# Joao-M-Silva/padel_analytics

Hardware: NVIDIA H100
Metric: frames/sec through trackers.runner (all 4 trackers) (higher is better)
Workload: dtype f16 storage, f32 accumulate

## Files before the change

padel_analytics_b200/csrc/api.cu:

```cuda
#include <atomic>
#include <cstring>
#include <map>
#include <memory>
#include <mutex>
#include <vector>

#include "internal.h"

namespace pb {

static thread_local std::string g_error;
std::atomic<long long> g_launches{0};

void set_error(const char* fmt, ...) {
  char buf[1024];
  va_list ap;
  va_start(ap, fmt);
  vsnprintf(buf, sizeof(buf), fmt, ap);
  va_end(ap);
  g_error = buf;
}

static std::atomic<int> g_plan_sm_limit{0};
static std::atomic<int> g_plan_pdl{-1};
// ... 145 lines not shown
  return -1;
}

int pb_program_op_info(const pb_program* p, int i, pb_op_info* out) {
  PB_CHECK(p && out, "program_op_info: null argument");
  PB_CHECK(i >= 0 && i < (int)p->ops.size(), "program_op_info: op %d out of range", i);
  const Op& op = p->ops[i];
  memset(out, 0, sizeof(*out));
  out->kernel = pb_program_op_kernel(p, i);
  if (op.kind == OpKind::Conv) {
    const ConvPlan& pl = *op.conv;
    const ConvKParams& kp = pl.kp;
    const pb_conv_desc& d = pl.desc;
    out->desc = d;
    out->variant = pl.variant != 1                ? PB_CONV_PER_TAP
                   : d.in_layout == PB_IN_STEM4   ? PB_CONV_STEM
                   : d.ksize == 1                 ? PB_CONV_HALO_1X1
                   : d.stride == 2                ? PB_CONV_HALO_S2
                                                  : PB_CONV_HALO;
    out->epi = pl.epi;
    out->BN = kp.BN;
    out->n_ntiles = kp.n_ntiles;
    out->KB = kp.KB;
    out->kblocks = kp.kblocks;
    if (pl.variant == 1) {
      out->S = kp.hs_S;
      out->G = kp.hs_G;
      out->b_resident = kp.b_resident;
      out->a_stages = kp.a_stages;
      out->b_stages = kp.b_stages;
      out->tma_store = kp.st_bytes != 0;
      out->st_pool = kp.st_pool;
    } else {
      out->S = 1;
      out->G = 1;
      out->a_stages = out->b_stages = kp.stages;
    }
    out->grid = pl.grid;
    out->total_tiles = kp.total_tiles;
    out->pdl = pl.pdl;
  } else {
    out->in = op.in;
    out->out = op.out;
    out->N = op.N;
    out->H = op.H;
    out->W = op.W;
    out->C = op.C;
    out->c_off = op.c_off;
    out->c = op.c;
    out->out_C = op.out_C;
    out->out_coff = op.out_coff;
    out->weight = op.hw;
    out->bias = op.hb;
  }
  return 0;
}

int pb_program_run_range(pb_program* p, int first, int last, void* stream) {
  PB_CHECK(p != nullptr, "program_run: null");
  PB_CHECK(first >= 0 && last <= (int)p->ops.size() && first <= last, "program_run: bad range");
  cudaStream_t s = static_cast<cudaStream_t>(stream);
  for (int i = first; i < last; ++i) {
    const Op& op = p->ops[i];
    int rc = 0;
    switch (op.kind) {
      case OpKind::Conv: rc = conv_plan_launch(op.conv.get(), s); break;
      case OpKind::MaxPool2:
        rc = launch_maxpool2(op.in, op.N, op.H, op.W, op.C, op.c_off, op.c, op.out, op.out_C, op.out_coff, s);
// ... 20 lines not shown
```

padel_analytics_b200/csrc/conv_tc.cu:

```cuda
#include <cstdlib>
#include <cstring>
#include <mutex>

#include "internal.h"
#include "ptx.cuh"
#include "conv_common.cuh"

namespace pb {

constexpr size_t kConvStageBudget = 196 * 1024;

struct ConvSmemTail {
  uint64_t full[kConvMaxStages];
  uint64_t empty[kConvMaxStages];
  float bias[kConvMaxCout];
  float scratch[kConvConsumerWarps * kEpiScratchFloats];
};

struct TileCoord {
  int nt, tw, th, tn;
};
__device__ __forceinline__ TileCoord decode_tile(const ConvKParams& kp, int tile) {
  TileCoord c;
  int t;
  fast_divmod(t, c.nt, tile, kp.fd_nt);
  fast_divmod(t, c.tw, t, kp.fd_w);
  fast_divmod(c.tn, c.th, t, kp.fd_h);
  return c;
}

template <int kEpi>
__global__ void __launch_bounds__(kConvThreads, 1)
conv_tc_kernel(const __grid_constant__ CUtensorMap tmap_a, const __grid_constant__ CUtensorMap tmap_w,
               const __grid_constant__ ConvKParams kp) {
  extern __shared__ __align__(1024) uint8_t smem_raw[];
  uint8_t* smem = smem_raw + ((1024u - (smem_u32(smem_raw) & 1023u)) & 1023u);
  const uint32_t stage_bytes = kp.a_bytes + kp.b_bytes;
  ConvSmemTail* tail = reinterpret_cast<ConvSmemTail*>(smem + (size_t)kp.stages * stage_bytes);

  const int warp = threadIdx.x >> 5;
  const int lane = threadIdx.x & 31;
  const int k_iters = kp.taps * kp.kblocks;

  if (warp == 0 && lane == 0) {
    tma_prefetch_desc(&tmap_a);
    for (int i = 0; i < kp.stages; ++i) {
      mbar_init(&tail->full[i], 2);
      mbar_init(&tail->empty[i], kConvConsumerWarps);
    }
    fence_mbar_init();
  }
  if (warp == 1 && lane == 0) tma_prefetch_desc(&tmap_w);
  for (int i = threadIdx.x; i < kp.cout_pad; i += blockDim.x) tail->bias[i] = kp.bias[i];
  __syncthreads();
  griddep_launch_dependents();
  if (warp != 1) griddep_wait();

  if (warp < 4) {
    warpgroup_reg_dealloc<kConvProducerRegs>();
    if (warp == 0 && lane == 0) {
      int stage = 0;
      uint32_t phase = 0;
      const int TW = 1 << kp.tw_log2, TH = 1 << kp.th_log2;
      const int TN = 128 >> (kp.tw_log2 + kp.th_log2);
      for (int tile = blockIdx.x; tile < kp.total_tiles; tile += gridDim.x) {
        const TileCoord tc = decode_tile(kp, tile);
        for (int tap = 0; tap < kp.taps; ++tap) {
          const int cw = tc.tw * TW + kp.tap_dw[tap];
          const int ch = tc.th * TH + kp.tap_dh[tap];
          const int cc = kp.c_in_off + kp.tap_dc[tap];
          for (int kb = 0; kb < kp.kblocks; ++kb) {
            mbar_wait(&tail->empty[stage], phase ^ 1);
            mbar_arrive_expect_tx(&tail->full[stage], kp.a_bytes);
            tma_load_5d(smem + (size_t)stage * stage_bytes, &tmap_a, &tail->full[stage], cc + kb * kp.KB, cw,
                        kp.tap_d2[tap], ch, tc.tn * TN);
            if (++stage == kp.stages) {
              stage = 0;
              phase ^= 1;
            }
          }
        }
      }
    } else if (warp == 1 && lane == 0) {
      int stage = 0;
      uint32_t phase = 0;
      for (int tile = blockIdx.x; tile < kp.total_tiles; tile += gridDim.x) {
        int nt, tq;
        fast_divmod(tq, nt, tile, kp.fd_nt);
        for (int tap = 0; tap < kp.taps; ++tap) {
          for (int kb = 0; kb < kp.kblocks; ++kb) {
            mbar_wait(&tail->empty[stage], phase ^ 1);
            mbar_arrive_expect_tx(&tail->full[stage], kp.b_tx_bytes);
            tma_load_3d(smem + (size_t)stage * stage_bytes + kp.a_bytes, &tmap_w, &tail->full[stage], kb * kp.KB,
                        nt * kp.BN, tap);
            if (++stage == kp.stages) {
              stage = 0;
              phase ^= 1;
            }
          }
        }
      }
    }
    return;
  }

  warpgroup_reg_alloc<kConvConsumerRegs>();
  const int cw = warp - 4, g = cw >> 2, wq = cw & 3;
  float* scr = tail->scratch + cw * kEpiScratchFloats;
  const uint32_t row_bytes = (uint32_t)kp.KB * 2u;
  const int ksteps = kp.KB / 16;
  const int p = 64 * g + 16 * wq + (lane & 15);
  const int TWm = (1 << kp.tw_log2) - 1, THm = (1 << kp.th_log2) - 1;
  const int tw_i = p & TWm;
  const int th_i = (p >> kp.tw_log2) & THm;
  const int tn_i = p >> (kp.tw_log2 + kp.th_log2);
  float acc[kConvAccRegs];
#pragma unroll
  for (int i = 0; i < kConvAccRegs; ++i) acc[i] = 0.f;
  int stage = 0;
  uint32_t phase = 0;
  for (int tile = blockIdx.x; tile < kp.total_tiles; tile += gridDim.x) {
    const TileCoord tc = decode_tile(kp, tile);
    int prev = -1;
    for (int it = 0; it < k_iters; ++it) {
      mbar_wait(&tail->full[stage], phase);
      const uint32_t a_addr = smem_u32(smem + (size_t)stage * stage_bytes) + 64u * (uint32_t)g * row_bytes;
      const uint64_t adesc = wgmma_desc_kmajor(a_addr, row_bytes);
      const uint64_t bdesc = wgmma_desc_kmajor(smem_u32(smem + (size_t)stage * stage_bytes + kp.a_bytes), row_bytes);
      wgmma_fence();
      for (int k = 0; k < ksteps; ++k)
        mma_group<1, 1>(kp.BN, acc, adesc + (uint64_t)(2 * k), 0, bdesc + (uint64_t)(2 * k), (uint32_t)((it | k) != 0));
      wgmma_commit();
      if (prev >= 0) {
        wgmma_wait<1>();
        consumer_release(&tail->empty[prev], lane);
      }
      prev = stage;
      if (++stage == kp.stages) {
        stage = 0;
        phase ^= 1;
      }
    }
    wgmma_wait<0>();
    wgmma_fence_operands(acc);
    consumer_release(&tail->empty[prev], lane);

    EpiPix px;
    px.ow = (tc.tw << kp.tw_log2) + tw_i;
    px.oh = (tc.th << kp.th_log2) + th_i;
    px.n = tc.tn * (128 >> (kp.tw_log2 + kp.th_log2)) + tn_i;
    px.valid = (px.ow < kp.Wo) && (px.oh < kp.Ho) && (px.n < kp.N);
    px.pix = ((size_t)px.n * kp.Ho + px.oh) * kp.Wo + px.ow;
    epilogue_tile<kEpi>(kp, acc, 1, tc.nt, tail->bias + tc.nt * kp.BN, scr, lane, [&](int, bool& pool_writer) {
      pool_writer = false;
      return px;
    });
  }
}

static EncodeTiledFn get_encode_fn() {
  static EncodeTiledFn fn = nullptr;
  static std::once_flag once;
  std::call_once(once, [] {
    void* p = nullptr;
    cudaDriverEntryPointQueryResult q;
    if (cudaGetDriverEntryPoint("cuTensorMapEncodeTiled", &p, cudaEnableDefault, &q) == cudaSuccess &&
        q == cudaDriverEntryPointSuccess)
      fn = reinterpret_cast<EncodeTiledFn>(p);
  });
  return fn;
}

static int ilog2(int v) {
  int l = 0;
  while ((1 << l) < v) ++l;
  return l;
}

int conv_epi_class(const pb_conv_desc* d, const ConvKParams& kp) {
  static const int enabled = [] {
    const char* e = getenv("PADEL_B200_CONV_EPI");
    return e ? atoi(e) : 1;
  }();
  if (!enabled || kp.dbg_flags != 0) return PB_EPI_GENERIC;
  if (d->head_n != 0 || d->out2_mode != PB_OUT2_NONE || (reinterpret_cast<uintptr_t>(d->out) & 31) != 0)
    return PB_EPI_GENERIC;
  if (d->out_mode == PB_OUT_F32_NHWC) {
// ... 78 lines not shown
  kp.res_first = d->res_before_act ? 1 : 0;
  kp.out = d->out;
  kp.out_C = d->out_C;
  kp.out_coff = d->out_coff;
  kp.out_mode = d->out_mode;
  kp.cout_store = d->cout_store;
  kp.out2 = d->out2;
  kp.out2_C = d->out2_C;
  kp.out2_coff = d->out2_coff;
  kp.out2_mode = d->out2_mode;
  kp.head_w = d->head_weight;
  kp.head_b = d->head_bias;
  kp.head_n = d->head_n;
  kp.head_out = d->head_out;
  {
    const char* df = getenv("PADEL_B200_CONV_DEBUG");
    kp.dbg_flags = df ? atoi(df) : 0;
  }
  plan->variant = 0;
  plan->pdl = plan_pdl();
  plan->epi = conv_epi_class(d, kp);
  if (stem) return conv_stem_setup(d, plan, encode);
  {
    const char* e = getenv("PADEL_B200_CONV_HALO");
    const int mode = e ? atoi(e) : 2;
    const bool s1_3x3 = d->ksize == 3 && d->stride == 1;
    if (mode == 1 || (mode == 2 && (d->cout_pad <= 192 || s1_3x3))) {
      const int rc = d->ksize == 1    ? conv_halo_1x1_setup(d, plan, encode)
                     : d->stride == 2 ? conv_halo_s2_setup(d, plan, encode)
                                      : conv_halo_setup(d, plan, encode, mode == 1 || d->out2_mode == PB_OUT2_POOL2);
      if (rc >= 0) return rc;
    }
  }
  PB_CHECK(d->out2_mode != PB_OUT2_POOL2,
           "conv: PB_OUT2_POOL2 is only implemented by the halo kernel (3x3 stride 1, cout <= 256 or a multiple of 128)");
  int nn = (d->cout_pad + 255) / 256;
  while (d->cout_pad % nn != 0 || (d->cout_pad / nn) % 16 != 0) ++nn;
  kp.n_ntiles = nn;
  kp.BN = d->cout_pad / nn;
  PB_CHECK(kp.BN >= 16 && kp.BN <= 256, "conv: cannot tile cout_pad %d", d->cout_pad);

  long best_cost = -1;
  int best_tw = 0, best_th = 0;
  for (int twl = 7; twl >= 2; --twl) {
    for (int thl = 7 - twl; thl >= 0; --thl) {
      const int TW = 1 << twl, TH = 1 << thl, TN = 128 >> (twl + thl);
      const long cost = (long)((kp.Wo + TW - 1) / TW) * ((kp.Ho + TH - 1) / TH) * ((kp.N + TN - 1) / TN);
      if (best_cost < 0 || cost < best_cost) {
        best_cost = cost;
        best_tw = twl;
        best_th = thl;
      }
    }
  }
  kp.tw_log2 = best_tw;
  kp.th_log2 = best_th;
  const int TW = 1 << best_tw, TH = 1 << best_th, TN = 128 >> (best_tw + best_th);
  kp.tiles_w = (kp.Wo + TW - 1) / TW;
  kp.tiles_h = (kp.Ho + TH - 1) / TH;
  kp.tiles_n = (kp.N + TN - 1) / TN;
  kp.total_tiles = kp.tiles_w * kp.tiles_h * kp.tiles_n * kp.n_ntiles;
  (void)ilog2;

  for (int r = 0; r < d->ksize; ++r)
    for (int q = 0; q < d->ksize; ++q) {
      const int t = r * d->ksize + q;
      const int dy = r - d->ksize / 2, dx = q - d->ksize / 2;
      if (s == 1) {
        kp.tap_dc[t] = 0;
        kp.tap_dw[t] = dx;
        kp.tap_d2[t] = 0;
        kp.tap_dh[t] = dy;
      } else {
        kp.tap_dw[t] = (dx < 0) ? -1 : 0;
        kp.tap_dc[t] = (dx != 0) ? d->C : 0;
        kp.tap_dh[t] = (dy < 0) ? -1 : 0;
        kp.tap_d2[t] = (dy != 0) ? 1 : 0;
      }
    }
  kp.a_bytes = 128u * kp.KB * 2u;
  kp.b_tx_bytes = (uint32_t)kp.BN * kp.KB * 2u;
  kp.b_bytes = (kp.b_tx_bytes + 1023u) & ~1023u;
  const uint32_t stage_bytes = kp.a_bytes + kp.b_bytes;
  int stages = (int)(kConvStageBudget / stage_bytes);
  if (stages > kConvMaxStages) stages = kConvMaxStages;
  PB_CHECK(stages >= 2, "conv: stage too large (%u bytes)", stage_bytes);
  kp.stages = stages;
  plan->smem_bytes = (size_t)stages * stage_bytes + sizeof(ConvSmemTail) + 1024;
  plan->threads = kConvThreads;
  plan->grid = kp.total_tiles < num_sms() ? kp.total_tiles : num_sms();
  const CUtensorMapSwizzle swz = kp.KB == 64   ? CU_TENSOR_MAP_SWIZZLE_128B
                                 : kp.KB == 32 ? CU_TENSOR_MAP_SWIZZLE_64B
                                               : CU_TENSOR_MAP_SWIZZLE_32B;
  {
    const cuuint64_t C = (cuuint64_t)d->C, W = (cuuint64_t)d->W, H = (cuuint64_t)d->H;
    cuuint64_t dims[5];
    cuuint64_t strides[4];
    if (s == 1) {
      dims[0] = C; dims[1] = W; dims[2] = 1; dims[3] = H; dims[4] = (cuuint64_t)d->N;
      strides[0] = C * 2; strides[1] = W * C * 2; strides[2] = W * C * 2; strides[3] = H * W * C * 2;
    } else {
      dims[0] = 2 * C; dims[1] = W / 2; dims[2] = 2; dims[3] = H / 2; dims[4] = (cuuint64_t)d->N;
      strides[0] = 2 * C * 2; strides[1] = W * C * 2; strides[2] = 2 * W * C * 2; strides[3] = H * W * C * 2;
    }
    cuuint32_t box[5] = {(cuuint32_t)kp.KB, (cuuint32_t)TW, 1, (cuuint32_t)TH, (cuuint32_t)TN};
    cuuint32_t estr[5] = {1, 1, 1, 1, 1};
    CUresult r = encode(&plan->tmap_a, CU_TENSOR_MAP_DATA_TYPE_FLOAT16, 5, const_cast<void*>(d->in), dims, strides,
                        box, estr, CU_TENSOR_MAP_INTERLEAVE_NONE, swz, CU_TENSOR_MAP_L2_PROMOTION_L2_128B,
                        CU_TENSOR_MAP_FLOAT_OOB_FILL_NONE);
    PB_CHECK(r == CUDA_SUCCESS, "conv: cuTensorMapEncodeTiled(A) failed with %d (N=%d H=%d W=%d C=%d s=%d)", (int)r,
             d->N, d->H, d->W, d->C, s);
  }
  {
    cuuint64_t dims[3] = {(cuuint64_t)d->cin, (cuuint64_t)d->cout_pad, (cuuint64_t)kp.taps};
    cuuint64_t strides[2] = {(cuuint64_t)d->cin * 2, (cuuint64_t)d->cin * d->cout_pad * 2};
    cuuint32_t box[3] = {(cuuint32_t)kp.KB, (cuuint32_t)kp.BN, 1};
    cuuint32_t estr[3] = {1, 1, 1};
    CUresult r = encode(&plan->tmap_w, CU_TENSOR_MAP_DATA_TYPE_FLOAT16, 3, const_cast<void*>(d->weight), dims,
                        strides, box, estr, CU_TENSOR_MAP_INTERLEAVE_NONE, swz, CU_TENSOR_MAP_L2_PROMOTION_L2_256B,
                        CU_TENSOR_MAP_FLOAT_OOB_FILL_NONE);
    PB_CHECK(r == CUDA_SUCCESS, "conv: cuTensorMapEncodeTiled(W) failed with %d", (int)r);
  }
  return 0;
}

int conv_plan_build(const pb_conv_desc* d, ConvPlan* plan) {
  const int rc = conv_plan_build_impl(d, plan);
  if (rc == 0) {
    plan->kp.fd_w = make_fastdiv(plan->kp.tiles_w);
    plan->kp.fd_h = make_fastdiv(plan->kp.tiles_h);
    plan->kp.fd_nt = make_fastdiv(plan->kp.n_ntiles);
  }
  return rc;
}

int conv_plan_launch(const ConvPlan* plan, cudaStream_t stream) {
  if (plan->variant == 1) return conv_halo_launch(plan, stream);
  typedef void (*TcKernelFn)(CUtensorMap, CUtensorMap, ConvKParams);
  const TcKernelFn fn = plan->epi == PB_EPI_SILU       ? conv_tc_kernel<PB_EPI_SILU>
                        : plan->epi == PB_EPI_RELU     ? conv_tc_kernel<PB_EPI_RELU>
                        : plan->epi == PB_EPI_SILU_RES ? conv_tc_kernel<PB_EPI_SILU_RES>
                        : plan->epi == PB_EPI_F32      ? conv_tc_kernel<PB_EPI_F32>
                                                       : conv_tc_kernel<PB_EPI_GENERIC>;
  PB_CUDA((cudaError_t)ensure_dynamic_smem(reinterpret_cast<const void*>(fn), 227 * 1024));
  PB_CUDA(launch_ex(fn, dim3(plan->grid), dim3(plan->threads), plan->smem_bytes, stream, 1, plan->pdl != 0, plan->tmap_a,
                    plan->tmap_w, plan->kp));
  count_launch();
  return 0;
}

__global__ void conv_reference_kernel(pb_conv_desc d, int Ho, int Wo) {
  const long total = (long)d.N * Ho * Wo * d.cout_pad;
  for (long idx = blockIdx.x * (long)blockDim.x + threadIdx.x; idx < total; idx += (long)gridDim.x * blockDim.x) {
    const int co = (int)(idx % d.cout_pad);
    long pixl = idx / d.cout_pad;
    const int ow = (int)(pixl % Wo);
    const int oh = (int)((pixl / Wo) % Ho);
    const int n = (int)(pixl / ((long)Wo * Ho));
    if (co >= d.cout_store) continue;
    const __half* in = reinterpret_cast<const __half*>(d.in);
    const __half* w = reinterpret_cast<const __half*>(d.weight);
    float acc = 0.f;
    const int pad = d.ksize / 2;
    for (int r = 0; r < d.ksize; ++r)
      for (int q = 0; q < d.ksize; ++q) {
        const int ih = oh * d.stride + r - pad, iw = ow * d.stride + q - pad;
        if (ih < 0 || ih >= d.H || iw < 0 || iw >= d.W) continue;
        if (d.in_layout == PB_IN_STEM4) {
          const __half* ip = in + (((size_t)n * (d.H + 2) + ih + 1) * (d.W + 2) + iw + 1) * 4;
          const __half* wp = w + ((size_t)r * d.cout_pad + co) * 16 + q * 4;
          for (int c = 0; c < 3; ++c) acc += __half2float(ip[c]) * __half2float(wp[c]);
          continue;
        }
        const __half* ip = in + (((size_t)n * d.H + ih) * d.W + iw) * d.C + d.c_in_off;
        const __half* wp = w + ((size_t)(r * d.ksize + q) * d.cout_pad + co) * d.cin;
        for (int c = 0; c < d.cin; ++c) acc += __half2float(ip[c]) * __half2float(wp[c]);
// ... 42 lines not shown
```

padel_analytics_b200/csrc/internal.h:

```cpp
#pragma once
#include <cuda.h>
#include <cuda_fp16.h>
#include <cuda_runtime.h>

#include <atomic>
#include <cstdarg>
#include <cstdlib>
#include <cstdio>
#include <string>

#include "../../include/padel_b200.h"

namespace pb {

void set_error(const char* fmt, ...);
extern std::atomic<long long> g_launches;
inline void count_launch(int n = 1) { g_launches.fetch_add(n, std::memory_order_relaxed); }
int num_sms();
int ensure_dynamic_smem(const void* func, size_t bytes);
bool pdl_enabled();
int plan_pdl();

#ifdef __CUDACC__
template <typename... KArgs, typename... Args>
// ... 78 lines not shown

struct ConvKParams {
  int N, Ho, Wo;
  int tiles_w, tiles_h, tiles_n, n_ntiles, total_tiles;
  FastDiv fd_w, fd_h, fd_nt;
  int tw_log2, th_log2;
  int taps, kblocks, KB, BN, stages, cout_pad;
  int c_in_off;
  int tap_dc[9], tap_dw[9], tap_d2[9], tap_dh[9];
  const float* bias;
  int act;
  const __half* res;
  int res_C, res_coff;
  int res_first;
  void* out;
  int out_C, out_coff, out_mode, cout_store;
  void* out2;
  int out2_C, out2_coff, out2_mode;
  uint32_t a_bytes, b_bytes, b_tx_bytes;
  const float* head_w;
  const float* head_b;
  int head_n;
  float* head_out;
  int b_resident;
  int hs_S, hs_P, hs_G, a_stages, b_stages;
  uint32_t halo_bytes;
  uint32_t hs_a_row_bytes;
  int hs_ntaps, hs_sbo_rows, hs_x0, hs_y0, hs_tile_h;
  int hs_tap_off[9];
  int hs_tap_desc[9];
  int dbg_flags;
  uint32_t st_bytes;
  int st_maps, st_pool;
};

constexpr int kHaloStoreMaps = 5;
struct HaloStoreMaps {
  CUtensorMap m[kHaloStoreMaps];
};

struct ConvPlan {
  pb_conv_desc desc;
  ConvKParams kp;
  CUtensorMap tmap_a;
  CUtensorMap tmap_w;
  HaloStoreMaps tmap_o;
  int grid;
  int threads;
  size_t smem_bytes;
  int variant;
  int pdl;
  int epi;
};

#define PB_EPI_GENERIC 0
#define PB_EPI_SILU 1
#define PB_EPI_RELU 2
#define PB_EPI_SILU_RES 3
#define PB_EPI_F32 4
int conv_epi_class(const pb_conv_desc* d, const ConvKParams& kp);

typedef CUresult (*EncodeTiledFn)(CUtensorMap*, CUtensorMapDataType, cuuint32_t, void*, const cuuint64_t*,
                                  const cuuint64_t*, const cuuint32_t*, const cuuint32_t*, CUtensorMapInterleave,
                                  CUtensorMapSwizzle, CUtensorMapL2promotion, CUtensorMapFloatOOBfill);
int conv_halo_setup(const pb_conv_desc* d, ConvPlan* plan, EncodeTiledFn encode, bool force);
int conv_stem_setup(const pb_conv_desc* d, ConvPlan* plan, EncodeTiledFn encode);
int conv_halo_s2_setup(const pb_conv_desc* d, ConvPlan* plan, EncodeTiledFn encode);
int conv_halo_1x1_setup(const pb_conv_desc* d, ConvPlan* plan, EncodeTiledFn encode);
int conv_halo_launch(const ConvPlan* plan, cudaStream_t stream);
int conv_plan_build(const pb_conv_desc* d, ConvPlan* plan);
int conv_plan_launch(const ConvPlan* plan, cudaStream_t stream);
int conv_reference_launch(const pb_conv_desc* d, cudaStream_t stream);

int launch_maxpool2(const void* in, int N, int H, int W, int C, int c_off, int c, void* out, int out_C,
                    int out_coff, cudaStream_t s);
int launch_upsample2(const void* in, int N, int H, int W, int C, int c_off, int c, void* out, int out_C,
                     int out_coff, cudaStream_t s);
int launch_sppf_pool(void* buf, int N, int H, int W, int C, int c, cudaStream_t s);
int launch_pointwise_head(const void* in, int N, int H, int W, int C, const float* w, const float* b, int n_out,
                          float* out, cudaStream_t s);

}
```

padel_analytics_b200/csrc/ptx.cuh:

```cuda
#pragma once
#include <cstdint>
#include <cuda.h>
#include <cuda_fp16.h>
#include <cuda_runtime.h>

namespace pb {

__device__ __forceinline__ uint32_t smem_u32(const void* p) {
  return static_cast<uint32_t>(__cvta_generic_to_shared(p));
}

__device__ __forceinline__ void mbar_init(uint64_t* bar, uint32_t count) {
  asm volatile("mbarrier.init.shared::cta.b64 [%0], %1;" ::"r"(smem_u32(bar)), "r"(count));
}
__device__ __forceinline__ void fence_mbar_init() {
  asm volatile("fence.mbarrier_init.release.cluster;" ::: "memory");
}
__device__ __forceinline__ void fence_proxy_async_smem() {
  asm volatile("fence.proxy.async.shared::cta;" ::: "memory");
}
__device__ __forceinline__ void mbar_arrive_expect_tx(uint64_t* bar, uint32_t bytes) {
  asm volatile("mbarrier.arrive.expect_tx.shared::cta.b64 _, [%0], %1;" ::"r"(smem_u32(bar)), "r"(bytes)
               : "memory");
}
__device__ __forceinline__ void mbar_arrive(uint64_t* bar) {
  asm volatile("mbarrier.arrive.shared::cta.b64 _, [%0];" ::"r"(smem_u32(bar)) : "memory");
}
__device__ __forceinline__ bool mbar_try_wait(uint64_t* bar, uint32_t parity) {
  uint32_t ok;
  asm volatile(
      "{\n\t.reg .pred p;\n\t"
      "mbarrier.try_wait.parity.shared::cta.b64 p, [%1], %2;\n\t"
      "selp.u32 %0, 1, 0, p;\n\t}"
      : "=r"(ok)
      : "r"(smem_u32(bar)), "r"(parity)
      : "memory");
  return ok != 0;
}
__device__ __forceinline__ void mbar_wait(uint64_t* bar, uint32_t parity) {
  while (!mbar_try_wait(bar, parity)) {
  }
}

__device__ __forceinline__ unsigned long long globaltimer_ns() {
  unsigned long long t;
  asm volatile("mov.u64 %0, %%globaltimer;" : "=l"(t));
  return t;
}
__device__ __forceinline__ void griddep_wait() { asm volatile("griddepcontrol.wait;" ::: "memory"); }
__device__ __forceinline__ void griddep_launch_dependents() {
  asm volatile("griddepcontrol.launch_dependents;" ::: "memory");
}

__device__ __forceinline__ void tma_prefetch_desc(const CUtensorMap* m) {
  asm volatile("prefetch.tensormap [%0];" ::"l"(reinterpret_cast<uint64_t>(m)) : "memory");
}
__device__ __forceinline__ void tma_load_3d(void* dst, const CUtensorMap* m, uint64_t* bar, int c0, int c1,
                                            int c2) {
  asm volatile(
      "cp.async.bulk.tensor.3d.shared::cluster.global.mbarrier::complete_tx::bytes [%0], [%1, {%3, %4, %5}], "
      "[%2];" ::"r"(smem_u32(dst)),
      "l"(reinterpret_cast<uint64_t>(m)), "r"(smem_u32(bar)), "r"(c0), "r"(c1), "r"(c2)
      : "memory");
}
__device__ __forceinline__ void tma_load_5d(void* dst, const CUtensorMap* m, uint64_t* bar, int c0, int c1,
                                            int c2, int c3, int c4) {
  asm volatile(
      "cp.async.bulk.tensor.5d.shared::cluster.global.mbarrier::complete_tx::bytes [%0], [%1, {%3, %4, %5, %6, "
      "%7}], [%2];" ::"r"(smem_u32(dst)),
      "l"(reinterpret_cast<uint64_t>(m)), "r"(smem_u32(bar)), "r"(c0), "r"(c1), "r"(c2), "r"(c3), "r"(c4)
      : "memory");
}

__device__ __forceinline__ void tma_store_4d(const CUtensorMap* m, const void* src, int c0, int c1, int c2, int c3) {
  asm volatile("cp.async.bulk.tensor.4d.global.shared::cta.bulk_group [%0, {%2, %3, %4, %5}], [%1];" ::"l"(
                   reinterpret_cast<uint64_t>(m)),
               "r"(smem_u32(src)), "r"(c0), "r"(c1), "r"(c2), "r"(c3)
               : "memory");
}
__device__ __forceinline__ void bulk_commit_group() { asm volatile("cp.async.bulk.commit_group;" ::: "memory"); }
__device__ __forceinline__ void bulk_wait_group_read0() {
  asm volatile("cp.async.bulk.wait_group.read 0;" ::: "memory");
}
__device__ __forceinline__ void bulk_wait_group0() { asm volatile("cp.async.bulk.wait_group 0;" ::: "memory"); }

__device__ __forceinline__ void named_barrier_sync(int id, int count) {
  asm volatile("bar.sync %0, %1;" ::"r"(id), "r"(count) : "memory");
}
// ... 129 lines not shown
```

padel_analytics_b200/engine/ops.py:

```python
from __future__ import annotations

import ctypes as C

import torch

from .. import _lib as L


def pad16(c: int) -> int:
    return (c + 15) // 16 * 16


def fold_bn(w: torch.Tensor, gamma, beta, mean, var, eps: float):
    scale = gamma / torch.sqrt(var + eps)
    return w * scale.reshape(-1, 1, 1, 1), beta - mean * scale


def pack_conv_weight(w: torch.Tensor, b: torch.Tensor | None, cin_pad: int, cout_pad: int, device,
                     cin_map: list[int] | None = None):
    cout, cin, kh, kw = w.shape
    assert kh == kw
    wp = torch.zeros(kh * kw, cout_pad, cin_pad, dtype=torch.float32)
    src = w.detach().float().permute(2, 3, 0, 1).reshape(kh * kw, cout, cin)
    if cin_map is None:
# ... 123 lines not shown
    def upsample2(self, x, c_off, c, out, out_coff):
        N, H, W, Ct = x.shape
        L.check(L.lib().pb_program_add_upsample2(self._h, x.data_ptr(), N, H, W, Ct, c_off, c, out.data_ptr(),
                                                 out.shape[-1], out_coff))
        self._note("up", N * H * W * c * 2 * 5.0)

    def sppf_pool(self, buf, c):
        N, H, W, Ct = buf.shape
        L.check(L.lib().pb_program_add_sppf_pool(self._h, buf.data_ptr(), N, H, W, Ct, c))
        self._note("sppf", N * H * W * c * 2 * 4.0)

    def pointwise_head(self, x, weight, bias, out):
        N, H, W, Ct = x.shape
        L.check(L.lib().pb_program_add_pointwise_head(self._h, x.data_ptr(), N, H, W, Ct, weight.data_ptr(),
                                                      bias.data_ptr(), weight.shape[0], out.data_ptr()))
        self.kinds.append("head")
        self.descs.append(None)
        self.flops.append(2.0 * N * H * W * Ct * weight.shape[0])
        self.bytes.append(float(N * H * W * (Ct * 2 + weight.shape[0] * 4)))

    def _note(self, kind: str, nbytes: float):
        self.kinds.append(kind)
        self.descs.append(None)
        self.flops.append(0.0)
        self.bytes.append(float(nbytes))

    @property
    def num_ops(self) -> int:
        return L.lib().pb_program_num_ops(self._h)

    def op_kernels(self) -> list[str]:
        names = {0: "conv_tc_kernel", 1: "conv_halo_kernel", 2: "maxpool2_kernel", 3: "upsample2_kernel",
                 4: "sppf_pool_kernel", 5: "pointwise_head_kernel"}
        return [names[L.lib().pb_program_op_kernel(self._h, i)] for i in range(self.num_ops)]

    def op_info(self, i: int) -> L.OpInfo:
        info = L.OpInfo()
        L.check(L.lib().pb_program_op_info(self._h, i, C.byref(info)))
        return info

    def run(self, first: int | None = None, last: int | None = None):
        if first is None:
            L.check(L.lib().pb_program_run(self._h, L.stream_ptr()))
        else:
            L.check(L.lib().pb_program_run_range(self._h, first, last, L.stream_ptr()))


def time_program_ops(prog: Program, repeats: int = 5):
    import statistics

    n = prog.num_ops
    samples = [[] for _ in range(n)]
    for _ in range(repeats):
        ev = [torch.cuda.Event(enable_timing=True) for _ in range(n + 1)]
        ev[0].record()
        for i in range(n):
            prog.run(i, i + 1)
            ev[i + 1].record()
        torch.cuda.synchronize()
        for i in range(n):
            samples[i].append(ev[i].elapsed_time(ev[i + 1]))
    return [statistics.median(s) for s in samples]
```

Before: 1357.

## Add weight-resident persistent 1x1 conv kernel for small head convolutions

Adds a specialized persistent wgmma kernel for 1x1 stride-1 convolutions with small cin/cout. It keeps the whole weight matrix resident in shared memory and streams 128-pixel activation tiles through a deep TMA ring. Two consumer warpgroups alternate tiles, and bias plus activation are fused into the epilogue. The aim is to cut per-tile weight reloads and pipeline overhead for head-style convs, at the cost of extra code paths and stricter eligibility checks.

```diff
diff --git a/padel_analytics_b200/csrc/api.cu b/padel_analytics_b200/csrc/api.cu
--- a/padel_analytics_b200/csrc/api.cu
+++ b/padel_analytics_b200/csrc/api.cu
@@ -203,6 +203,7 @@
     } else {
       out->S = 1;
       out->G = 1;
+      out->b_resident = pl.variant == 2;
       out->a_stages = out->b_stages = kp.stages;
     }
     out->grid = pl.grid;
diff --git a/padel_analytics_b200/csrc/conv_head.cu b/padel_analytics_b200/csrc/conv_head.cu
--- /dev/null
+++ b/padel_analytics_b200/csrc/conv_head.cu
@@ -0,0 +1,287 @@
+#include <cstdlib>
+
+#include "internal.h"
+#include "ptx.cuh"
+#include "conv_common.cuh"
+
+namespace pb {
+
+constexpr int kHeadTile = 128;
+constexpr int kHeadMaxStages = 16;
+constexpr int kHeadMaxCin = 192;
+constexpr int kHeadMaxCout = 128;
+constexpr size_t kHeadSmemBudget = 200 * 1024;
+
+struct HeadSmemTail {
+  uint64_t full[kHeadMaxStages];
+  uint64_t empty[kHeadMaxStages];
+  uint64_t bank;
+  float bias[kHeadMaxCout];
+};
+
+template <int kBN>
+__global__ void __launch_bounds__(kConvThreads, 1)
+conv_head_kernel(const __grid_constant__ CUtensorMap tmap_a, const __grid_constant__ CUtensorMap tmap_w,
+                 const __grid_constant__ ConvKParams kp) {
+  extern __shared__ __align__(1024) uint8_t smem_raw[];
+  uint8_t* smem = smem_raw + ((1024u - (smem_u32(smem_raw) & 1023u)) & 1023u);
+  uint8_t* bank = smem;
+  uint8_t* ring = smem + (size_t)kp.kblocks * kp.b_bytes;
+  HeadSmemTail* tail = reinterpret_cast<HeadSmemTail*>(ring + (size_t)kp.stages * kp.a_bytes);
+  const uint32_t kb_bytes = (uint32_t)kHeadTile * kp.KB * 2u;
+
+  const int warp = threadIdx.x >> 5;
+  const int lane = threadIdx.x & 31;
+  if (warp == 0 && lane == 0) {
+    tma_prefetch_desc(&tmap_a);
+    tma_prefetch_desc(&tmap_w);
+    for (int i = 0; i < kp.stages; ++i) {
+      mbar_init(&tail->full[i], 1);
+      mbar_init(&tail->empty[i], kConvConsumerWarps / 2);
+    }
+    mbar_init(&tail->bank, 1);
+    fence_mbar_init();
+  }
+  for (int i = threadIdx.x; i < kp.cout_pad; i += blockDim.x) tail->bias[i] = kp.bias[i];
+  __syncthreads();
+  griddep_launch_dependents();
+
+  if (warp < 4) {
+    warpgroup_reg_dealloc<kConvProducerRegs>();
+    if (warp == 0 && lane == 0) {
+      mbar_arrive_expect_tx(&tail->bank, (uint32_t)kp.kblocks * kp.b_tx_bytes);
+      for (int kb = 0; kb < kp.kblocks; ++kb)
+        tma_load_2d(bank + (size_t)kb * kp.b_bytes, &tmap_w, &tail->bank, kb * kp.KB, 0);
+      griddep_wait();
+      int stage = 0;
+      uint32_t phase = 0;
+      for (int tile = blockIdx.x; tile < kp.total_tiles; tile += gridDim.x) {
+        mbar_wait(&tail->empty[stage], phase ^ 1);
+        mbar_arrive_expect_tx(&tail->full[stage], kp.a_bytes);
+        uint8_t* dst = ring + (size_t)stage * kp.a_bytes;
+        for (int kb = 0; kb < kp.kblocks; ++kb)
+          tma_load_2d(dst + (size_t)kb * kb_bytes, &tmap_a, &tail->full[stage], kp.c_in_off + kb * kp.KB,
+                      tile * kHeadTile);
+        if (++stage == kp.stages) {
+          stage = 0;
+          phase ^= 1;
+        }
+      }
+    }
+    return;
+  }
+
+  warpgroup_reg_alloc<kConvConsumerRegs>();
+  griddep_wait();
+  const int g = (warp - 4) >> 2, wq = warp & 3;
+  const uint32_t row_bytes = (uint32_t)kp.KB * 2u;
+  const int ksteps = kp.KB / 16;
+  const int HW = kp.Ho * kp.Wo;
+  const int npix = kp.N * HW;
+  const bool sigmoid = kp.act == PB_ACT_SIGMOID;
+  const bool silu = kp.act == PB_ACT_SILU;
+  const bool f16 = kp.out_mode == PB_OUT_F16_NHWC;
+  const bool nchw = kp.out_mode == PB_OUT_F32_NCHW;
+  const int r0 = 16 * wq + (lane >> 2);
+  const int q = lane & 3;
+  const uint32_t bank_addr = smem_u32(bank);
+  float acc[kBN];
+#pragma unroll
+  for (int i = 0; i < kBN; ++i) acc[i] = 0.f;
+  mbar_wait(&tail->bank, 0);
+
+  int stage = g, phase = 0;
+  for (int tile = blockIdx.x + g * gridDim.x; tile < kp.total_tiles; tile += 2 * gridDim.x) {
+    if (stage >= kp.stages) {
+      stage -= kp.stages;
+      phase ^= 1;
+    }
+    mbar_wait(&tail->full[stage], (uint32_t)phase);
+    const uint32_t a_addr = smem_u32(ring + (size_t)stage * kp.a_bytes);
+    wgmma_fence();
+    for (int kb = 0; kb < kp.kblocks; ++kb) {
+      const uint64_t ad = wgmma_desc_kmajor(a_addr + (uint32_t)kb * kb_bytes, row_bytes);
+      const uint64_t bd = wgmma_desc_kmajor(bank_addr + (uint32_t)kb * kp.b_bytes, row_bytes);
+      const uint64_t half = (uint64_t)((64u * row_bytes) >> 4);
+      for (int k = 0; k < ksteps; ++k) {
+        const uint32_t accum = (uint32_t)((kb | k) != 0);
+        wgmma_f16<kBN>(acc, ad + (uint64_t)(2 * k), bd + (uint64_t)(2 * k), accum);
+        wgmma_f16<kBN>(acc + kBN / 2, ad + half + (uint64_t)(2 * k), bd + (uint64_t)(2 * k), accum);
+      }
+    }
+    wgmma_commit();
+    wgmma_wait<0>();
+    wgmma_fence_operands(acc);
+    consumer_release(&tail->empty[stage], lane);
+    stage += 2;
+
+    if (f16) {
+      __half* out = reinterpret_cast<__half*>(kp.out);
+#pragma unroll
+      for (int j = 0; j < 2; ++j) {
+#pragma unroll
+        for (int h = 0; h < 2; ++h) {
+          const int p = tile * kHeadTile + 64 * j + r0 + 8 * h;
+          __half* op = out + (size_t)p * kp.out_C + kp.out_coff;
+#pragma unroll
+          for (int i = 0; i < kBN / 8; i += 2) {
+            if (8 * i >= kp.cout_store) break;
+            const int c = 8 * i + 2 * q;
+            const float2 b0 = *reinterpret_cast<const float2*>(tail->bias + c);
+            const float2 b1 = *reinterpret_cast<const float2*>(tail->bias + c + 8);
+            float v0 = acc[kBN / 2 * j + 4 * i + 2 * h] + b0.x;
+            float v1 = acc[kBN / 2 * j + 4 * i + 2 * h + 1] + b0.y;
+            float v2 = acc[kBN / 2 * j + 4 * i + 4 + 2 * h] + b1.x;
+            float v3 = acc[kBN / 2 * j + 4 * i + 4 + 2 * h + 1] + b1.y;
+            if (silu) {
+              silu2_frag(v0, v1);
+              silu2_frag(v2, v3);
+            } else {
+              v0 = fmaxf(v0, 0.f);
+              v1 = fmaxf(v1, 0.f);
+              v2 = fmaxf(v2, 0.f);
+              v3 = fmaxf(v3, 0.f);
+            }
+            const __half2 h01 = __floats2half2_rn(v0, v1), h23 = __floats2half2_rn(v2, v3);
+            const uint32_t w0 = *reinterpret_cast<const uint32_t*>(&h01);
+            const uint32_t w1 = *reinterpret_cast<const uint32_t*>(&h23);
+            const uint32_t got = __shfl_xor_sync(0xffffffffu, (q & 1) ? w0 : w1, 1);
+            if (p < npix) {
+              if (q & 1)
+                *reinterpret_cast<uint2*>(op + c + 6) = make_uint2(got, w1);
+              else
+                *reinterpret_cast<uint2*>(op + c) = make_uint2(w0, got);
+            }
+          }
+        }
+      }
+      continue;
+    }
+    float* out = reinterpret_cast<float*>(kp.out);
+#pragma unroll
+    for (int j = 0; j < 2; ++j) {
+#pragma unroll
+      for (int h = 0; h < 2; ++h) {
+        const int p = tile * kHeadTile + 64 * j + r0 + 8 * h;
+        if (p >= npix) continue;
+        size_t base, cstride;
+        if (nchw) {
+          int n, hw;
+          fast_divmod(n, hw, p, kp.fd_hw);
+          base = (size_t)n * kp.cout_store * HW + hw;
+          cstride = (size_t)HW;
+        } else {
+          base = (size_t)p * kp.out_C + kp.out_coff;
+          cstride = 1;
+        }
+#pragma unroll
+        for (int i = 0; i < kBN / 8; ++i) {
+          if (8 * i >= kp.cout_store) break;
+          const int c = 8 * i + 2 * q;
+          const float2 b = *reinterpret_cast<const float2*>(tail->bias + c);
+          float v0 = acc[kBN / 2 * j + 4 * i + 2 * h] + b.x;
+          float v1 = acc[kBN / 2 * j + 4 * i + 2 * h + 1] + b.y;
+          if (sigmoid) {
+            v0 = __fdividef(1.f, 1.f + __expf(-v0));
+            v1 = __fdividef(1.f, 1.f + __expf(-v1));
+          }
+          if (nchw) {
+            out[base + (size_t)c * cstride] = v0;
+            out[base + (size_t)(c + 1) * cstride] = v1;
+          } else {
+            *reinterpret_cast<float2*>(out + base + c) = make_float2(v0, v1);
+          }
+        }
+      }
+    }
+  }
+}
+
+int conv_head_setup(const pb_conv_desc* d, ConvPlan* plan, EncodeTiledFn encode) {
+  static const int enabled = [] {
+    const char* e = getenv("PADEL_B200_CONV_HEAD");
+    return e ? atoi(e) : 1;
+  }();
+  if (!enabled || d->in_layout != PB_IN_NHWC || d->ksize != 1 || d->stride != 1 || d->res || d->head_n != 0 ||
+      d->out2_mode != PB_OUT2_NONE)
+    return -1;
+  if (d->out_mode == PB_OUT_F16_NHWC) {
+    if (plan->epi != PB_EPI_SILU && plan->epi != PB_EPI_RELU) return -1;
+  } else if (d->out_mode == PB_OUT_F32_NHWC || d->out_mode == PB_OUT_F32_NCHW) {
+    if (d->act != PB_ACT_NONE && d->act != PB_ACT_SIGMOID) return -1;
+  } else {
+    return -1;
+  }
+  if (d->cin > kHeadMaxCin || d->cout_pad > kHeadMaxCout || d->cout_store % 8 != 0) return -1;
+  if (d->out_mode == PB_OUT_F32_NHWC &&
+      (((d->out_C | d->out_coff) & 7) != 0 || d->out_coff + d->cout_store > d->out_C))
+    return -1;
+  if ((reinterpret_cast<uintptr_t>(d->out) & 31) != 0) return -1;
+  const long npix = (long)d->N * d->H * d->W;
+  if (npix + kHeadTile >= (1l << 31)) return -1;
+
+  ConvKParams& kp = plan->kp;
+  kp.BN = d->cout_pad;
+  kp.n_ntiles = 1;
+  kp.total_tiles = (int)((npix + kHeadTile - 1) / kHeadTile);
+  kp.tiles_w = kp.total_tiles;
+  kp.tiles_h = kp.tiles_n = 1;
+  kp.fd_hw = make_fastdiv(kp.Ho * kp.Wo);
+  kp.a_bytes = (uint32_t)kHeadTile * d->cin * 2u;
+  kp.b_tx_bytes = (uint32_t)kp.BN * kp.KB * 2u;
+  kp.b_bytes = (kp.b_tx_bytes + 1023u) & ~1023u;
+  const size_t bank_bytes = (size_t)kp.kblocks * kp.b_bytes;
+  int stages = (int)((kHeadSmemBudget - bank_bytes) / kp.a_bytes);
+  kp.stages = stages < kHeadMaxStages ? stages : kHeadMaxStages;
+  PB_CHECK(kp.stages >= 2, "conv(head): %d-byte tiles leave room for %d stages", kp.a_bytes, kp.stages);
+  plan->smem_bytes = bank_bytes + (size_t)kp.stages * kp.a_bytes + sizeof(HeadSmemTail) + 1024;
+  plan->threads = kConvThreads;
+  plan->grid = kp.total_tiles < num_sms() ? kp.total_tiles : num_sms();
+  plan->variant = 2;
+  const CUtensorMapSwizzle swz = kp.KB == 64   ? CU_TENSOR_MAP_SWIZZLE_128B
+                                 : kp.KB == 32 ? CU_TENSOR_MAP_SWIZZLE_64B
+                                               : CU_TENSOR_MAP_SWIZZLE_32B;
+  {
+    cuuint64_t dims[2] = {(cuuint64_t)d->C, (cuuint64_t)npix};
+    cuuint64_t strides[1] = {(cuuint64_t)d->C * 2};
+    cuuint32_t box[2] = {(cuuint32_t)kp.KB, (cuuint32_t)kHeadTile};
+    cuuint32_t estr[2] = {1, 1};
+    CUresult r = encode(&plan->tmap_a, CU_TENSOR_MAP_DATA_TYPE_FLOAT16, 2, const_cast<void*>(d->in), dims, strides,
+                        box, estr, CU_TENSOR_MAP_INTERLEAVE_NONE, swz, CU_TENSOR_MAP_L2_PROMOTION_L2_128B,
+                        CU_TENSOR_MAP_FLOAT_OOB_FILL_NONE);
+    PB_CHECK(r == CUDA_SUCCESS, "conv(head): cuTensorMapEncodeTiled(A) failed with %d (pixels %ld, C %d)", (int)r,
+             npix, d->C);
+  }
+  {
+    cuuint64_t dims[2] = {(cuuint64_t)d->cin, (cuuint64_t)d->cout_pad};
+    cuuint64_t strides[1] = {(cuuint64_t)d->cin * 2};
+    cuuint32_t box[2] = {(cuuint32_t)kp.KB, (cuuint32_t)kp.BN};
+    cuuint32_t estr[2] = {1, 1};
+    CUresult r = encode(&plan->tmap_w, CU_TENSOR_MAP_DATA_TYPE_FLOAT16, 2, const_cast<void*>(d->weight), dims,
+                        strides, box, estr, CU_TENSOR_MAP_INTERLEAVE_NONE, swz, CU_TENSOR_MAP_L2_PROMOTION_L2_256B,
+                        CU_TENSOR_MAP_FLOAT_OOB_FILL_NONE);
+    PB_CHECK(r == CUDA_SUCCESS, "conv(head): cuTensorMapEncodeTiled(W) failed with %d", (int)r);
+  }
+  return 0;
+}
+
+int conv_head_launch(const ConvPlan* plan, cudaStream_t stream) {
+  typedef void (*HeadKernelFn)(CUtensorMap, CUtensorMap, ConvKParams);
+  HeadKernelFn fn = nullptr;
+  switch (plan->kp.BN) {
+#define PB_HEAD_CASE(n_) \
+  case n_: fn = conv_head_kernel<n_>; break;
+    PB_HEAD_CASE(16) PB_HEAD_CASE(32) PB_HEAD_CASE(48) PB_HEAD_CASE(64) PB_HEAD_CASE(80) PB_HEAD_CASE(96)
+    PB_HEAD_CASE(112) PB_HEAD_CASE(128)
+#undef PB_HEAD_CASE
+    default: break;
+  }
+  PB_CHECK(fn != nullptr, "conv(head): no kernel instantiation for N=%d", plan->kp.BN);
+  PB_CUDA((cudaError_t)ensure_dynamic_smem(reinterpret_cast<const void*>(fn), 227 * 1024));
+  PB_CUDA(launch_ex(fn, dim3(plan->grid), dim3(plan->threads), plan->smem_bytes, stream, 1, plan->pdl != 0,
+                    plan->tmap_a, plan->tmap_w, plan->kp));
+  count_launch();
+  return 0;
+}
+
+}
diff --git a/padel_analytics_b200/csrc/conv_tc.cu b/padel_analytics_b200/csrc/conv_tc.cu
--- a/padel_analytics_b200/csrc/conv_tc.cu
+++ b/padel_analytics_b200/csrc/conv_tc.cu
@@ -297,6 +297,10 @@
       if (rc >= 0) return rc;
     }
   }
+  {
+    const int rc = conv_head_setup(d, plan, encode);
+    if (rc >= 0) return rc;
+  }
   PB_CHECK(d->out2_mode != PB_OUT2_POOL2,
            "conv: PB_OUT2_POOL2 is only implemented by the halo kernel (3x3 stride 1, cout <= 256 or a multiple of 128)");
   int nn = (d->cout_pad + 255) / 256;
@@ -401,6 +405,7 @@
 
 int conv_plan_launch(const ConvPlan* plan, cudaStream_t stream) {
   if (plan->variant == 1) return conv_halo_launch(plan, stream);
+  if (plan->variant == 2) return conv_head_launch(plan, stream);
   typedef void (*TcKernelFn)(CUtensorMap, CUtensorMap, ConvKParams);
   const TcKernelFn fn = plan->epi == PB_EPI_SILU       ? conv_tc_kernel<PB_EPI_SILU>
                         : plan->epi == PB_EPI_RELU     ? conv_tc_kernel<PB_EPI_RELU>
diff --git a/padel_analytics_b200/csrc/internal.h b/padel_analytics_b200/csrc/internal.h
--- a/padel_analytics_b200/csrc/internal.h
+++ b/padel_analytics_b200/csrc/internal.h
@@ -134,6 +134,7 @@
   int dbg_flags;
   uint32_t st_bytes;
   int st_maps, st_pool;
+  FastDiv fd_hw;
 };
 
 constexpr int kHaloStoreMaps = 5;
@@ -170,6 +171,8 @@
 int conv_halo_s2_setup(const pb_conv_desc* d, ConvPlan* plan, EncodeTiledFn encode);
 int conv_halo_1x1_setup(const pb_conv_desc* d, ConvPlan* plan, EncodeTiledFn encode);
 int conv_halo_launch(const ConvPlan* plan, cudaStream_t stream);
+int conv_head_setup(const pb_conv_desc* d, ConvPlan* plan, EncodeTiledFn encode);
+int conv_head_launch(const ConvPlan* plan, cudaStream_t stream);
 int conv_plan_build(const pb_conv_desc* d, ConvPlan* plan);
 int conv_plan_launch(const ConvPlan* plan, cudaStream_t stream);
 int conv_reference_launch(const pb_conv_desc* d, cudaStream_t stream);
diff --git a/padel_analytics_b200/csrc/ptx.cuh b/padel_analytics_b200/csrc/ptx.cuh
--- a/padel_analytics_b200/csrc/ptx.cuh
+++ b/padel_analytics_b200/csrc/ptx.cuh
@@ -54,6 +54,13 @@
 
 __device__ __forceinline__ void tma_prefetch_desc(const CUtensorMap* m) {
   asm volatile("prefetch.tensormap [%0];" ::"l"(reinterpret_cast<uint64_t>(m)) : "memory");
+}
+__device__ __forceinline__ void tma_load_2d(void* dst, const CUtensorMap* m, uint64_t* bar, int c0, int c1) {
+  asm volatile(
+      "cp.async.bulk.tensor.2d.shared::cluster.global.mbarrier::complete_tx::bytes [%0], [%1, {%3, %4}], [%2];" ::"r"(
+          smem_u32(dst)),
+      "l"(reinterpret_cast<uint64_t>(m)), "r"(smem_u32(bar)), "r"(c0), "r"(c1)
+      : "memory");
 }
 __device__ __forceinline__ void tma_load_3d(void* dst, const CUtensorMap* m, uint64_t* bar, int c0, int c1,
                                             int c2) {
diff --git a/padel_analytics_b200/engine/ops.py b/padel_analytics_b200/engine/ops.py
--- a/padel_analytics_b200/engine/ops.py
+++ b/padel_analytics_b200/engine/ops.py
@@ -179,7 +179,11 @@
     def op_kernels(self) -> list[str]:
         names = {0: "conv_tc_kernel", 1: "conv_halo_kernel", 2: "maxpool2_kernel", 3: "upsample2_kernel",
                  4: "sppf_pool_kernel", 5: "pointwise_head_kernel"}
-        return [names[L.lib().pb_program_op_kernel(self._h, i)] for i in range(self.num_ops)]
+        out = []
+        for i in range(self.num_ops):
+            k = L.lib().pb_program_op_kernel(self._h, i)
+            out.append("conv_head_kernel" if k == 0 and self.op_info(i).b_resident else names[k])
+        return out
 
     def op_info(self, i: int) -> L.OpInfo:
         info = L.OpInfo()
```

New measurement: 1401 (median of 6 runs). 3.3% higher.

## Batch multiple pixel sub-tiles per weight load in per-tap conv kernel

Applied to the files above, without the earlier changes.

The per-tap tensor-core conv kernel can now process kS pixel sub-tiles (up to 4) per CTA tile. It loads one weight block per stage and reuses it across several A tiles via compile-time templated MMA and epilogue. The planner turns this on only for 1x1, stride-1 convs without a second output, and only when the estimated makespan gets at most 10% worse. This amortizes weight traffic and per-tile overhead, at the cost of more shared memory per stage (fewer stages), more template instantiations and more accumulator registers.

```diff
diff --git a/padel_analytics_b200/csrc/api.cu b/padel_analytics_b200/csrc/api.cu
--- a/padel_analytics_b200/csrc/api.cu
+++ b/padel_analytics_b200/csrc/api.cu
@@ -201,7 +201,7 @@
       out->tma_store = kp.st_bytes != 0;
       out->st_pool = kp.st_pool;
     } else {
-      out->S = 1;
+      out->S = kp.hs_S;
       out->G = 1;
       out->a_stages = out->b_stages = kp.stages;
     }
diff --git a/padel_analytics_b200/csrc/conv_tc.cu b/padel_analytics_b200/csrc/conv_tc.cu
--- a/padel_analytics_b200/csrc/conv_tc.cu
+++ b/padel_analytics_b200/csrc/conv_tc.cu
@@ -13,34 +13,35 @@
 struct ConvSmemTail {
   uint64_t full[kConvMaxStages];
   uint64_t empty[kConvMaxStages];
-  float bias[kConvMaxCout];
-  float scratch[kConvConsumerWarps * kEpiScratchFloats];
+  alignas(16) float bias[kConvMaxCout];
+  alignas(16) float scratch[kConvConsumerWarps * kEpiScratchFloats];
 };
 
 struct TileCoord {
-  int nt, tw, th, tn;
+  int tw, th, tn;
 };
-__device__ __forceinline__ TileCoord decode_tile(const ConvKParams& kp, int tile) {
+__device__ __forceinline__ TileCoord decode_group(const ConvKParams& kp, int group) {
   TileCoord c;
   int t;
-  fast_divmod(t, c.nt, tile, kp.fd_nt);
-  fast_divmod(t, c.tw, t, kp.fd_w);
+  fast_divmod(t, c.tw, group, kp.fd_w);
   fast_divmod(c.tn, c.th, t, kp.fd_h);
   return c;
 }
 
-template <int kEpi>
+template <int kEpi, int kS, int kBN>
 __global__ void __launch_bounds__(kConvThreads, 1)
 conv_tc_kernel(const __grid_constant__ CUtensorMap tmap_a, const __grid_constant__ CUtensorMap tmap_w,
                const __grid_constant__ ConvKParams kp) {
   extern __shared__ __align__(1024) uint8_t smem_raw[];
   uint8_t* smem = smem_raw + ((1024u - (smem_u32(smem_raw) & 1023u)) & 1023u);
-  const uint32_t stage_bytes = kp.a_bytes + kp.b_bytes;
+  const uint32_t a_stage_bytes = (uint32_t)kS * kp.a_bytes;
+  const uint32_t stage_bytes = a_stage_bytes + kp.b_bytes;
   ConvSmemTail* tail = reinterpret_cast<ConvSmemTail*>(smem + (size_t)kp.stages * stage_bytes);
 
   const int warp = threadIdx.x >> 5;
   const int lane = threadIdx.x & 31;
   const int k_iters = kp.taps * kp.kblocks;
+  const int groups = kp.tiles_w * kp.tiles_h * kp.tiles_n;
 
   if (warp == 0 && lane == 0) {
     tma_prefetch_desc(&tmap_a);
@@ -64,16 +65,24 @@
       const int TW = 1 << kp.tw_log2, TH = 1 << kp.th_log2;
       const int TN = 128 >> (kp.tw_log2 + kp.th_log2);
       for (int tile = blockIdx.x; tile < kp.total_tiles; tile += gridDim.x) {
-        const TileCoord tc = decode_tile(kp, tile);
+        int gt, nt;
+        fast_divmod(gt, nt, tile, kp.fd_nt);
+        TileCoord tc[kS];
+#pragma unroll
+        for (int j = 0; j < kS; ++j) {
+          const int grp = gt * kS + j;
+          tc[j] = decode_group(kp, grp < groups ? grp : groups - 1);
+        }
         for (int tap = 0; tap < kp.taps; ++tap) {
-          const int cw = tc.tw * TW + kp.tap_dw[tap];
-          const int ch = tc.th * TH + kp.tap_dh[tap];
           const int cc = kp.c_in_off + kp.tap_dc[tap];
           for (int kb = 0; kb < kp.kblocks; ++kb) {
             mbar_wait(&tail->empty[stage], phase ^ 1);
-            mbar_arrive_expect_tx(&tail->full[stage], kp.a_bytes);
-            tma_load_5d(smem + (size_t)stage * stage_bytes, &tmap_a, &tail->full[stage], cc + kb * kp.KB, cw,
-                        kp.tap_d2[tap], ch, tc.tn * TN);
+            mbar_arrive_expect_tx(&tail->full[stage], a_stage_bytes);
+#pragma unroll
+            for (int j = 0; j < kS; ++j)
+              tma_load_5d(smem + (size_t)stage * stage_bytes + (size_t)j * kp.a_bytes, &tmap_a, &tail->full[stage],
+                          cc + kb * kp.KB, tc[j].tw * TW + kp.tap_dw[tap], kp.tap_d2[tap],
+                          tc[j].th * TH + kp.tap_dh[tap], tc[j].tn * TN);
             if (++stage == kp.stages) {
               stage = 0;
               phase ^= 1;
@@ -91,7 +100,7 @@
           for (int kb = 0; kb < kp.kblocks; ++kb) {
             mbar_wait(&tail->empty[stage], phase ^ 1);
             mbar_arrive_expect_tx(&tail->full[stage], kp.b_tx_bytes);
-            tma_load_3d(smem + (size_t)stage * stage_bytes + kp.a_bytes, &tmap_w, &tail->full[stage], kb * kp.KB,
+            tma_load_3d(smem + (size_t)stage * stage_bytes + a_stage_bytes, &tmap_w, &tail->full[stage], kb * kp.KB,
                         nt * kp.BN, tap);
             if (++stage == kp.stages) {
               stage = 0;
@@ -114,22 +123,32 @@
   const int tw_i = p & TWm;
   const int th_i = (p >> kp.tw_log2) & THm;
   const int tn_i = p >> (kp.tw_log2 + kp.th_log2);
-  float acc[kConvAccRegs];
+  const uint64_t sub_units = (uint64_t)(kp.a_bytes >> 4);
+  static_assert(kBN > 0 || kS == 1, "several sub-tiles need a compile-time N tile");
+  constexpr int kNch = (kBN + 31) / 32;
+  constexpr int kAcc = kBN > 0 ? kS * kNch * 16 : kConvAccRegs;
+  static_assert(kAcc <= kConvAccRegs, "accumulators of kS sub-tiles must fit the registers");
+  float acc[kAcc];
 #pragma unroll
-  for (int i = 0; i < kConvAccRegs; ++i) acc[i] = 0.f;
+  for (int i = 0; i < kAcc; ++i) acc[i] = 0.f;
   int stage = 0;
   uint32_t phase = 0;
   for (int tile = blockIdx.x; tile < kp.total_tiles; tile += gridDim.x) {
-    const TileCoord tc = decode_tile(kp, tile);
+    int gt, nt;
+    fast_divmod(gt, nt, tile, kp.fd_nt);
     int prev = -1;
     for (int it = 0; it < k_iters; ++it) {
       mbar_wait(&tail->full[stage], phase);
       const uint32_t a_addr = smem_u32(smem + (size_t)stage * stage_bytes) + 64u * (uint32_t)g * row_bytes;
       const uint64_t adesc = wgmma_desc_kmajor(a_addr, row_bytes);
-      const uint64_t bdesc = wgmma_desc_kmajor(smem_u32(smem + (size_t)stage * stage_bytes + kp.a_bytes), row_bytes);
+      const uint64_t bdesc = wgmma_desc_kmajor(smem_u32(smem + (size_t)stage * stage_bytes + a_stage_bytes), row_bytes);
       wgmma_fence();
       for (int k = 0; k < ksteps; ++k)
-        mma_group<1, 1>(kp.BN, acc, adesc + (uint64_t)(2 * k), 0, bdesc + (uint64_t)(2 * k), (uint32_t)((it | k) != 0));
+        if constexpr (kBN > 0)
+          mma_n<kBN, kS, 1>(acc, adesc + (uint64_t)(2 * k), sub_units, bdesc + (uint64_t)(2 * k),
+                            (uint32_t)((it | k) != 0));
+        else
+          mma_group<1, 1>(kp.BN, acc, adesc + (uint64_t)(2 * k), 0, bdesc + (uint64_t)(2 * k), (uint32_t)((it | k) != 0));
       wgmma_commit();
       if (prev >= 0) {
         wgmma_wait<1>();
@@ -145,14 +164,17 @@
     wgmma_fence_operands(acc);
     consumer_release(&tail->empty[prev], lane);
 
-    EpiPix px;
-    px.ow = (tc.tw << kp.tw_log2) + tw_i;
-    px.oh = (tc.th << kp.th_log2) + th_i;
-    px.n = tc.tn * (128 >> (kp.tw_log2 + kp.th_log2)) + tn_i;
-    px.valid = (px.ow < kp.Wo) && (px.oh < kp.Ho) && (px.n < kp.N);
-    px.pix = ((size_t)px.n * kp.Ho + px.oh) * kp.Wo + px.ow;
-    epilogue_tile<kEpi>(kp, acc, 1, tc.nt, tail->bias + tc.nt * kp.BN, scr, lane, [&](int, bool& pool_writer) {
+    const float* sbias = tail->bias + nt * kp.BN;
+    epilogue_tile<kEpi, (kBN > 0 ? kS : 0), kNch>(kp, acc, kS, nt, sbias, scr, lane, [&](int j, bool& pool_writer) {
       pool_writer = false;
+      const int grp = gt * kS + j;
+      const TileCoord tc = decode_group(kp, grp);
+      EpiPix px;
+      px.ow = (tc.tw << kp.tw_log2) + tw_i;
+      px.oh = (tc.th << kp.th_log2) + th_i;
+      px.n = tc.tn * (128 >> (kp.tw_log2 + kp.th_log2)) + tn_i;
+      px.valid = grp < groups && (px.ow < kp.Wo) && (px.oh < kp.Ho) && (px.n < kp.N);
+      px.pix = ((size_t)px.n * kp.Ho + px.oh) * kp.Wo + px.ow;
       return px;
     });
   }
@@ -324,7 +346,6 @@
   kp.tiles_w = (kp.Wo + TW - 1) / TW;
   kp.tiles_h = (kp.Ho + TH - 1) / TH;
   kp.tiles_n = (kp.N + TN - 1) / TN;
-  kp.total_tiles = kp.tiles_w * kp.tiles_h * kp.tiles_n * kp.n_ntiles;
   (void)ilog2;
 
   for (int r = 0; r < d->ksize; ++r)
@@ -346,7 +367,18 @@
   kp.a_bytes = 128u * kp.KB * 2u;
   kp.b_tx_bytes = (uint32_t)kp.BN * kp.KB * 2u;
   kp.b_bytes = (kp.b_tx_bytes + 1023u) & ~1023u;
-  const uint32_t stage_bytes = kp.a_bytes + kp.b_bytes;
+  kp.hs_S = 1;
+  if (d->ksize == 1 && s == 1 && d->out2_mode == PB_OUT2_NONE) {
+    const long groups = (long)kp.tiles_w * kp.tiles_h * kp.tiles_n, sms = num_sms();
+    auto makespan = [&](long S) { return ((groups + S - 1) / S * kp.n_ntiles + sms - 1) / sms * S; };
+    const bool inst = plan->epi == PB_EPI_SILU || plan->epi == PB_EPI_F32 || plan->epi == PB_EPI_GENERIC;
+    for (int S = kp.BN <= 64 ? 4 : 2; inst && kp.BN <= 128 && S >= 2 && kp.hs_S == 1; S >>= 1) {
+      const size_t sb = (size_t)S * kp.a_bytes + kp.b_bytes;
+      if (kConvStageBudget / sb >= 3 && 10 * makespan(S) <= 11 * makespan(1)) kp.hs_S = S;
+    }
+  }
+  kp.total_tiles = (int)((kp.tiles_w * kp.tiles_h * kp.tiles_n + kp.hs_S - 1) / kp.hs_S) * kp.n_ntiles;
+  const uint32_t stage_bytes = (uint32_t)kp.hs_S * kp.a_bytes + kp.b_bytes;
   int stages = (int)(kConvStageBudget / stage_bytes);
   if (stages > kConvMaxStages) stages = kConvMaxStages;
   PB_CHECK(stages >= 2, "conv: stage too large (%u bytes)", stage_bytes);
@@ -399,14 +431,38 @@
   return rc;
 }
 
+typedef void (*TcKernelFn)(CUtensorMap, CUtensorMap, ConvKParams);
+
+template <int kEpi>
+static TcKernelFn tc_kernel_multi(int S, int BN) {
+#define PB_TC_BN(s_, n_) \
+  if (S == s_ && BN == n_) return conv_tc_kernel<kEpi, s_, n_>;
+  PB_TC_BN(4, 16) PB_TC_BN(4, 32) PB_TC_BN(4, 48) PB_TC_BN(4, 64)
+  PB_TC_BN(2, 16) PB_TC_BN(2, 32) PB_TC_BN(2, 48) PB_TC_BN(2, 64)
+  PB_TC_BN(2, 80) PB_TC_BN(2, 96) PB_TC_BN(2, 112) PB_TC_BN(2, 128)
+#undef PB_TC_BN
+  return nullptr;
+}
+
+static TcKernelFn tc_kernel_pick(int epi, int S, int BN) {
+  if (S > 1) {
+    return epi == PB_EPI_SILU  ? tc_kernel_multi<PB_EPI_SILU>(S, BN)
+           : epi == PB_EPI_F32 ? tc_kernel_multi<PB_EPI_F32>(S, BN)
+           : epi == PB_EPI_GENERIC ? tc_kernel_multi<PB_EPI_GENERIC>(S, BN)
+                                   : nullptr;
+  }
+  return epi == PB_EPI_SILU       ? conv_tc_kernel<PB_EPI_SILU, 1, 0>
+         : epi == PB_EPI_RELU     ? conv_tc_kernel<PB_EPI_RELU, 1, 0>
+         : epi == PB_EPI_SILU_RES ? conv_tc_kernel<PB_EPI_SILU_RES, 1, 0>
+         : epi == PB_EPI_F32      ? conv_tc_kernel<PB_EPI_F32, 1, 0>
+                                  : conv_tc_kernel<PB_EPI_GENERIC, 1, 0>;
+}
+
 int conv_plan_launch(const ConvPlan* plan, cudaStream_t stream) {
   if (plan->variant == 1) return conv_halo_launch(plan, stream);
-  typedef void (*TcKernelFn)(CUtensorMap, CUtensorMap, ConvKParams);
-  const TcKernelFn fn = plan->epi == PB_EPI_SILU       ? conv_tc_kernel<PB_EPI_SILU>
-                        : plan->epi == PB_EPI_RELU     ? conv_tc_kernel<PB_EPI_RELU>
-                        : plan->epi == PB_EPI_SILU_RES ? conv_tc_kernel<PB_EPI_SILU_RES>
-                        : plan->epi == PB_EPI_F32      ? conv_tc_kernel<PB_EPI_F32>
-                                                       : conv_tc_kernel<PB_EPI_GENERIC>;
+  const TcKernelFn fn = tc_kernel_pick(plan->epi, plan->kp.hs_S, plan->kp.BN);
+  PB_CHECK(fn != nullptr, "conv: no per-tap kernel instantiation for S=%d, N=%d, epilogue class %d", plan->kp.hs_S,
+           plan->kp.BN, plan->epi);
   PB_CUDA((cudaError_t)ensure_dynamic_smem(reinterpret_cast<const void*>(fn), 227 * 1024));
   PB_CUDA(launch_ex(fn, dim3(plan->grid), dim3(plan->threads), plan->smem_bytes, stream, 1, plan->pdl != 0, plan->tmap_a,
                     plan->tmap_w, plan->kp));
```

Result: faster. 1366 before, 1402 after (median of 6 runs) (+2.6%).
